# gmlwns2000/sharkshark-4k

Hardware: AMD Instinct MI355X
Metric: upscaled frames/sec at 720p->1440p x2 (whole job) (higher is better)
Workload: dtype f16; 1 GPU; RealESRGAN RRDBNet x2 (23 blocks) 720p->1440p fp16 [BASELINE configs[2]]; io=uint8 NHWC resident in HBM

## Files before the change

### sharkshark-4k_amd/csrc/common.h

```cpp
#pragma once
#include <hip/hip_runtime.h>
#include <hip/hip_fp16.h>
#include <algorithm>
#include <cstdint>
#include <cstdio>
#include <cstdlib>
#include <cstring>
#include <map>
#include <tuple>
#include <set>
#include <string>
#include <vector>
#include <stdexcept>
#include "../../include/ss4k.h"
#ifdef SS4K_DEV
#include "../../include/ss4k_dev.h"
#endif

namespace ss4k {

void set_error(const char* fmt, ...);

struct Error : std::runtime_error {
  int code;
// ... 177 lines not shown

struct ConvArgs {
  const char* in0; size_t in0_plane_bytes; int in0_plane0, nchunks0;
  const char* in1; size_t in1_plane_bytes; int in1_plane0, nchunks1;
  const char* zero_page;
  int N, H, W;
  int n0;
  int job_n;
  float grid_share;
  int mb_override;
  int wide_rl;
  int wide;
  int no_band;
  int ups2;
  int ups_presum;
  const void* wpk;
  const void* w16;
  const float* bias;
  const float* prelu;
  int prelu_le1;
  int act; float slope;
  float alpha, gamma;
  const char* res1; size_t r1_plane_bytes; int r1_plane0;
  const char* res2; size_t r2_plane_bytes; int r2_plane0;
  int bsvd_resid;
  int epi;
  char* out; size_t out_plane_bytes; int out_plane0;
  int cout_real, cout_pad;
  int tiles_x, tiles_y;
  int reverse;
  double flops;
  int dbg;
  unsigned long long* dbg_buf;
};
inline double conv_plane_span_f16(const ConvArgs& a) { return (double)std::max(a.n0 + a.N, a.job_n) * a.H * a.W * 32.0; }
enum { DBG_NO_STORE = 1, DBG_NO_MMA = 2, DBG_NO_TILE_DMA = 4, DBG_NO_W_DMA = 8, DBG_NO_EPILOGUE = 16, DBG_STAMP = 32 };

void launch_conv3x3(ss4k_ctx* ctx, const ConvArgs& a, int dtype, hipStream_t st);
struct PairArgs {
  const char* in; size_t in_plane_bytes; int in_plane0, planes_a;
  const char* wA; const float* biasA;
  const char* wB; const float* biasB;
  const char* res; size_t res_plane_bytes; int res_plane0;
  const char* zero_page;
  unsigned long long* dbg_buf;
  char* out; size_t out_plane_bytes; int out_plane0;
  int epi;
  int cout_real;
  int n0, N, H, W, bands;
  float grid_share;
  double flops;
};
inline bool conv3x3_pair_eligible(int planes_a, int cout_pad_a, int nchunks_b, int cout_pad_b) {
  return (planes_a == 1 || planes_a == 2) && cout_pad_a == 32 && nchunks_b == 2 && cout_pad_b == 32;
}
void launch_conv3x3_pair(ss4k_ctx* ctx, const PairArgs& a, hipStream_t st);

struct DenseArgs {
  const char* in0; size_t in0_plane_bytes; int in0_plane0, nchunks0;
  const char* in1; size_t in1_plane_bytes; int in1_plane0, nchunks1;
  const char* w1; const float* bias1;
  const char* w2; const float* bias2;
  float slope;
  char* out1; size_t out1_plane_bytes; int out1_plane0;
  char* out2; size_t out2_plane_bytes; int out2_plane0;
  const char* zero_page;
// ... 4 lines not shown
  unsigned long long* dbg_buf;
};
inline bool conv3x3_dense2_eligible(int nchunks_a, int cout_pad_a, int nchunks_b, int cout_pad_b) {
  return cout_pad_a == 32 && cout_pad_b == 32 && nchunks_b == nchunks_a + 2 && nchunks_a >= 2 && nchunks_a % 2 == 0;
}
struct ConvArgs;
bool conv3x3_wide_eligible(const ConvArgs& a, int dtype);
void launch_conv3x3_wide(ss4k_ctx* ctx, const ConvArgs& a, hipStream_t st);
void launch_conv3x3_dense2(ss4k_ctx* ctx, const DenseArgs& a, hipStream_t st);
bool conv3x3_w16_eligible(const ConvArgs& a, int dtype);
void launch_conv3x3_w16(ss4k_ctx* ctx, const ConvArgs& a, hipStream_t st);
bool conv3x3_w16n_eligible(const ConvArgs& a, int dtype);
void launch_conv3x3_w16n(ss4k_ctx* ctx, const ConvArgs& a, hipStream_t st);

inline int conv_cw(int) { return 16; }
inline int cout_pad_of(int cout) { return cout <= 32 ? 32 : (cout + 63) / 64 * 64; }
inline int conv_rec_bytes(int dtype) { return dtype == SS4K_F16 ? 32 : 64; }

struct PackSpec {
  int dtype;
  int cout_real, cin_total;
  std::vector<int> cin_map;
  int nchunks0, nchunks1;
  int ps2;
};
struct PackedConv {
  std::vector<uint8_t> w;
  std::vector<float> bias, prelu;
  int cout_pad, nb, groups;
};
PackedConv pack_conv3x3(const PackSpec& s, const float* w_oihw, const float* bias, const float* prelu);
std::vector<uint8_t> pack_conv3x3_w16(const PackSpec& s, const float* w_oihw, int cout_pad);
std::vector<uint8_t> pack_conv3x3_w16n(const PackSpec& s, const float* w_oihw);
int virt_to_real_cout(const PackSpec& s, int v);

}
```

### sharkshark-4k_amd/csrc/conv_dense.hip

```cpp
#include "common.h"
#include <cmath>
#include "conv_tile.h"

namespace ss4k {
namespace dense {

constexpr int NW = 4, MB = 4, TH = NW * MB;
constexpr int XH = TH + 4, XW = TW + 4;
constexpr int REC = 32, SPR = 2;
constexpr int ROWX = XW * REC;
constexpr int XT_SLOTS = XH * XW * SPR;
constexpr int XT_BYTES = XT_SLOTS * 16;
constexpr int XT_DMA = (XT_SLOTS + 63) / 64;
constexpr int DMA_PER_WAVE = (XT_DMA + NW - 1) / NW;
constexpr int WU = 6 * 1024, NSLOT = 5;
constexpr int NDMA = 11;
constexpr int W_OFF = 2 * XT_BYTES, B_OFF = W_OFF + NSLOT * WU, R_OFF = B_OFF + 64 * 4;
constexpr size_t LDS_BYTES = R_OFF + 64 * NW * 4;
static_assert(2 * LDS_BYTES <= 160 * 1024, "two workgroups per CU");
static_assert((TH + 3) * ROWX <= XT_BYTES, "x_k's plane image fits a tile buffer");

__constant__ uint32_t RING_TAB[128] = {
  0x10000, 0x10f00, 0x11000, 0x11500, 0x10300, 0x10400, 0x10600, 0x10a00, 0x11d00, 0x11e00, 0x10005, 0x12106, 0x11600, 0x11900, 0x12100, 0x10003,
  0x12107, 0x1000a, 0x1000c, 0x10511, 0x12108, 0x10009, 0x10111, 0x10611, 0x11311, 0x11611, 0x11d11, 0x00000, 0x10911, 0x10a11, 0x10b11, 0x11111,
// ... 331 lines not shown
      }
    }
    stamp(10);
    if (next_tile < 0) break;
    tile = next_tile; ++kt;
  }
  if constexpr (STAMP) {
    if (lane == 0 && a.dbg_buf && blockIdx.x < 1024) {
      unsigned long long* o = a.dbg_buf + ((size_t)blockIdx.x * 4 + wave) * 16;
      for (int k = 0; k < 11; ++k) o[k] = ph[k];
      o[11] = (unsigned long long)(kt + 1);
      o[12] = ((__builtin_amdgcn_s_memtime() - ct0) << 20) / (__builtin_amdgcn_s_memrealtime() - rt0 + 1);
    }
  }
}

}

namespace wide {

constexpr int NW = 4, MB = 4, TH = NW * MB;
constexpr int XH = TH + 2, XW = TW + 2;
constexpr int REC = 32, SPR = 2;
constexpr int ROWX = XW * REC;
constexpr int XT_SLOTS = XH * XW * SPR;
constexpr int XT_BYTES = XT_SLOTS * 16;
constexpr int XT_DMA = (XT_SLOTS + 63) / 64;
constexpr int DMA_PER_WAVE = (XT_DMA + NW - 1) / NW;
constexpr int WU = 6 * 1024, NSLOT = 6;
constexpr int NDMA = DMA_PER_WAVE + 5;
constexpr int W_OFF = 2 * XT_BYTES, B_OFF = W_OFF + NSLOT * WU;
constexpr size_t LDS_BYTES = B_OFF + 2 * 64 * 4;
static_assert(2 * LDS_BYTES <= 160 * 1024, "two workgroups per CU");

template <bool UPS, bool RL = false>
__global__ __launch_bounds__(64 * NW, 2) void conv3x3_wide_kernel(const ConvArgs a) {
  extern __shared__ __attribute__((aligned(16))) char smem[];
  const uint32_t lds0 = (uint32_t)(size_t)(__attribute__((address_space(3))) char*)smem;
  const int tid = threadIdx.x, lane = tid & 63;
  const int wave = __builtin_amdgcn_readfirstlane(tid >> 6);
  const int lr = lane & 31, lh = lane >> 5;
  const int grp = blockIdx.y;
  const int K = a.nchunks0 + a.nchunks1;
  const int ntiles = a.N * a.tiles_y * a.tiles_x;
  const char* wbase = reinterpret_cast<const char*>(a.wpk) + (size_t)grp * K * (3 * WU);
  const int Hs = a.ups2 ? (a.H >> 1) : a.H, Ws = a.ups2 ? (a.W >> 1) : a.W;

  const bool banded = (gridDim.x % 8 == 0) && ntiles >= (int)gridDim.x && !a.no_band;
  const int tpx = (ntiles + 7) / 8;
  auto tile_of = [&](int k) -> int {
    if (!banded) {
      const int t = blockIdx.x + k * gridDim.x;
      return t < ntiles ? (a.reverse ? ntiles - 1 - t : t) : -1;
    }
    const int base = (blockIdx.x & 7) * tpx, len = min(tpx, ntiles - base);
    const int j = (blockIdx.x >> 3) + k * (gridDim.x >> 3);
    return j < len ? base + (a.reverse ? len - 1 - j : j) : -1;
  };
  auto swz = [](int x) { return (x >> 3) & 1; };
  int rd_base[3];
#pragma unroll
  for (int dx = 0; dx < 3; ++dx) { const int c = lr + dx; rd_base[dx] = (((wave * MB) * XW + c) * SPR + (lh ^ swz(c))) * 16; }

  uint32_t src_off[DMA_PER_WAVE];
  auto setup_tile = [&](int tile, int& n, int& y0, int& x0) {
    const int tx = tile % a.tiles_x, tyn = tile / a.tiles_x;
// ... 229 lines not shown
            }
            __builtin_amdgcn_sched_barrier(0);
            float v[16], r1[16], r2[16];
#pragma unroll
            for (int hq = 0; hq < 2; ++hq) {
              load8<__half>(reinterpret_cast<const char*>(&r1v[hq]), r1 + 8 * hq);
              load8<__half>(reinterpret_cast<const char*>(&r2v[hq]), r2 + 8 * hq);
            }
#pragma unroll
            for (int i = 0; i < 16; ++i) {
              float t = acc[nb][mb][i];
              const float neg = t * slope_v[i];
              t = t >= 0.f ? t : neg;
              if (a.act == ACT_RELU6) t = fminf(t, 6.f);
              t = t * alpha + r1[i];
              v[i] = t * gamma + r2[i];
            }
            if (ok) {
              char* o = outp + rec;
              store8<__half>(o, v);
              store8<__half>(o + a.out_plane_bytes, v + 8);
            }
            __builtin_amdgcn_sched_barrier(0);
          }
        }
        __builtin_amdgcn_sched_barrier(0);
      }
    }
    if (next_tile < 0) break;
    tile = next_tile; ++kt;
  }
}

}

bool conv3x3_wide_eligible(const ConvArgs& a, int dtype) {
  return dtype == SS4K_F16 && a.epi == EPI_NHWC && !a.bsvd_resid && !a.dbg && a.cout_pad >= 64 && a.cout_pad % 64 == 0 &&
         conv_plane_span_f16(a) < 4294967296.0 && (!a.ups2 || (a.H % 2 == 0 && a.W % 2 == 0));
}

void launch_conv3x3_wide(ss4k_ctx* ctx, const ConvArgs& a0, hipStream_t st) {
  using namespace wide;
  ConvArgs a = a0;
  a.tiles_x = (a.W + TW - 1) / TW; a.tiles_y = (a.H + TH - 1) / TH;
  a.zero_page = ctx->zero_page();
  const int groups = a.cout_pad / 64;
  const int ntiles = a.N * a.tiles_y * a.tiles_x;
  const int gx = std::min(ntiles, std::max(1, (int)(ctx->num_cu * 2 / groups * (a.grid_share > 0.f ? a.grid_share : 1.f))));
  auto go = [&](auto kern) {
    const void* fn = reinterpret_cast<const void*>(kern);
    if (ctx->lds_attr_set.insert(fn).second)
      SS4K_HIP(hipFuncSetAttribute(fn, hipFuncAttributeMaxDynamicSharedMemorySize, (int)LDS_BYTES));
    hipLaunchKernelGGL(kern, dim3(gx, groups), dim3(64 * NW), LDS_BYTES, st, a);
  };
  const bool alpha_exact = a.alpha != 0.f && std::fabs(__half2float(__float2half(1.f / a.alpha)) * a.alpha - 1.f) <= 1.2e-7f;
  const bool rl = a.wide_rl && a.res1 && a.act == ACT_NONE && alpha_exact && a.nchunks0 == 4 && a.cout_pad == 64 && !a.ups2 &&
                  a.res1 + (size_t)a.r1_plane0 * a.r1_plane_bytes == a.in0 + (size_t)a.in0_plane0 * a.in0_plane_bytes &&
                  a.r1_plane_bytes == a.in0_plane_bytes;
  ctx->prof_family = rl ? "wide::conv3x3_wide_kernel<RL> (64-cout tile, 32x32x16 MFMA, residual through the matrix core)"
                     : (a.ups2 && a.ups_presum) ? "wide::conv3x3_wide_kernel<UPS> (64-cout tile, 32x32x16 MFMA, nearest-x2 input, pre-summed row taps)"
                                                : "wide::conv3x3_wide_kernel (64-cout tile, 32x32x16 MFMA)";
  if (rl) go(&conv3x3_wide_kernel<false, true>);
  else if (a.ups2 && a.ups_presum) go(&conv3x3_wide_kernel<true>);
  else go(&conv3x3_wide_kernel<false>);
  SS4K_HIP(hipGetLastError());
}

void launch_conv3x3_dense2(ss4k_ctx* ctx, const DenseArgs& a0, hipStream_t st) {
  using namespace dense;
  DenseArgs a = a0;
  SS4K_REQUIRE(a.N > 0 && a.H > 0 && a.W > 0, "dense pair: empty grid");
  SS4K_REQUIRE((a.nchunks0 + a.nchunks1) % 2 == 0 && a.nchunks0 + a.nchunks1 >= 2, "dense pair: conv_k needs an even number of K-chunks");
  SS4K_REQUIRE(a.slope >= 0.f && a.slope <= 1.f, "dense pair: LeakyReLU slope must be in [0,1]");
  SS4K_REQUIRE((double)(a.n0 + a.N) * a.H * a.W * 32.0 < 4294967296.0, "dense pair: a plane holds at most 4 GB");
  a.tiles_x = (a.W + TW - 1) / TW; a.tiles_y = (a.H + TH - 1) / TH;
  a.zero_page = ctx->zero_page();
  const int ntiles = a.N * a.tiles_y * a.tiles_x;
  int gx = std::min(ntiles, std::max(1, (int)(ctx->num_cu * 2 * (a.grid_share > 0.f ? a.grid_share : 1.f))));
#ifdef SS4K_DEV
  if (const char* e = std::getenv("SS4K_DENSE_GRID")) gx = std::min(ntiles, std::max(1, std::atoi(e)));
#endif
  ProfScope prof(ctx, st, PROF_CONV);
  auto go = [&](auto kern) {
    const void* fn = reinterpret_cast<const void*>(kern);
    if (ctx->lds_attr_set.insert(fn).second)
      SS4K_HIP(hipFuncSetAttribute(fn, hipFuncAttributeMaxDynamicSharedMemorySize, (int)LDS_BYTES));
    hipLaunchKernelGGL(kern, dim3(gx), dim3(64 * NW), LDS_BYTES, st, a);
  };
#ifdef SS4K_DEV
  static const bool stamp_mode = std::getenv("SS4K_DENSE_STAMP") && std::getenv("SS4K_DENSE_STAMP")[0] == '1';
  if (stamp_mode) {
    static unsigned long long* dbuf = nullptr;
    if (!dbuf) SS4K_HIP(hipMalloc(reinterpret_cast<void**>(&dbuf), 1024 * 4 * 16 * 8));
    SS4K_HIP(hipMemsetAsync(dbuf, 0, 1024 * 4 * 16 * 8, st));
    a.dbg_buf = dbuf;
    go(&conv3x3_dense2_kernel<0, true>);
// ... 39 lines not shown
```

### sharkshark-4k_amd/csrc/models.cpp

```cpp
#include "models.h"
#include <algorithm>
#include <cmath>
#include <cstdlib>
#include <cstring>

namespace ss4k {

static size_t esz(int dtype) { return dtype == SS4K_F16 ? 2 : 4; }
static int pad16(int c) { return (c + 15) / 16 * 16; }


static std::vector<std::pair<int, int>> bsvd_denblock_shapes(const int* chns, int in_ch, int out_ch, int interm) {
  const int c0 = chns[0], c1 = chns[1], c2 = chns[2];
  return {{interm, in_ch}, {c0, interm}, {c1, c0}, {c1, c1}, {c1, c1}, {c2, c1}, {c2, c2}, {c2, c2},
          {c2, c2}, {c2, c2}, {c1 * 4, c2}, {c1, c1}, {c1, c1}, {c0 * 4, c1}, {c0, c0}, {out_ch, c0}};
}

static void validate_desc(const ss4k_model_desc& d);

size_t model_param_count(const ss4k_model_desc& d) {
  try { validate_desc(d); } catch (const Error&) { return 0; }
  switch (d.kind) {
    case SS4K_FSRCNN:
      return 56 * 25 + 56 + 56 + 12 * 56 + 12 + 12 + 4 * (12 * 12 * 9 + 12 + 12) + 56 * 12 + 56 + 56 + 56 * 81 + 1;
// ... 38 lines not shown
  SS4K_REQUIRE(d.bsvd_stream == 0 || (d.bsvd_stream == 1 && d.kind == SS4K_BSVD), "desc.bsvd_stream is 0 or 1 and only applies to BSVD");
  switch (d.kind) {
    case SS4K_FSRCNN:
      SS4K_REQUIRE(d.scale == 2 || d.scale == 4, "FSRCNN scale must be 2 or 4");
      break;
    case SS4K_RRDBNET:
      SS4K_REQUIRE(d.scale == 1 || d.scale == 2 || d.scale == 4, "RRDBNet scale must be 1, 2 or 4");
      SS4K_REQUIRE(width(d.num_feat, 32), "RRDBNet: num_feat must be a multiple of 32 in 32..512");
      SS4K_REQUIRE(width(d.num_grow_ch, 32), "RRDBNet: num_grow_ch must be a multiple of 32 in 32..512");
      SS4K_REQUIRE(d.num_block > 0 && d.num_block <= MAX_BLOCKS, "RRDBNet: num_block must be in 1..64");
      break;
    case SS4K_SRVGG:
      SS4K_REQUIRE(d.scale == 2 || d.scale == 4, "SRVGG upscale must be 2 or 4 (PixelShuffle tail)");
      SS4K_REQUIRE(width(d.num_feat, 16), "SRVGG: num_feat must be a multiple of 16 in 16..512");
      SS4K_REQUIRE(d.num_block >= 0 && d.num_block <= MAX_BLOCKS, "SRVGG: num_block must be in 0..64");
      break;
    case SS4K_BSVD:
      SS4K_REQUIRE(width(d.bsvd_chns[0], 32), "BSVD: bsvd_chns[0] must be a multiple of 32 in 32..512");
      SS4K_REQUIRE(width(d.bsvd_chns[1], 64), "BSVD: bsvd_chns[1] must be a multiple of 64 in 64..512");
      SS4K_REQUIRE(width(d.bsvd_chns[2], 64), "BSVD: bsvd_chns[2] must be a multiple of 64 in 64..512");
      SS4K_REQUIRE(width(d.bsvd_mid_ch, 32), "BSVD: bsvd_mid_ch must be a multiple of 32 in 32..512");
      SS4K_REQUIRE(d.bsvd_interm_ch > 0 && d.bsvd_interm_ch <= 256, "BSVD: bsvd_interm_ch must be in 1..256");
      break;
    default:
      throw Error(SS4K_EINVAL, "unknown model kind");
  }
}

static void upload(DevBuf& b, const void* src, size_t bytes) {
  b.ensure(std::max<size_t>(bytes, 16));
  SS4K_HIP(hipMemcpy(b.ptr, src, bytes, hipMemcpyHostToDevice));
}

int Model::add_conv(ParamCursor& pc, int cout, int cin_total, PackSpec s, bool has_prelu_after) {
  s.dtype = desc.dtype; s.cout_real = cout; s.cin_total = cin_total;
  const float* w = pc.take((size_t)cout * cin_total * 9);
  const float* b = pc.take(cout);
  const float* a = has_prelu_after ? pc.take(cout) : nullptr;
  PackedConv p = pack_conv3x3(s, w, b, a);
  ConvLayer L;
  upload(L.w, p.w.data(), p.w.size());
  upload(L.bias, p.bias.data(), p.bias.size() * 4);
  if (a) upload(L.prelu, p.prelu.data(), p.prelu.size() * 4);
  if (use_w16 && use_wide && desc.dtype == SS4K_F16 && p.nb == 2 && p.cout_pad % 64 == 0 && (s.nchunks0 + s.nchunks1) % 2 == 0 && !s.ps2) {
    const std::vector<uint8_t> w6 = pack_conv3x3_w16(s, w, p.cout_pad);
    upload(L.w16, w6.data(), w6.size());
    weight_bytes += w6.size();
  }
  if (use_w16 && desc.dtype == SS4K_F16 && cout <= 4 && (s.nchunks0 + s.nchunks1) % 2 == 0 && !s.ps2) {
    const std::vector<uint8_t> w6 = pack_conv3x3_w16n(s, w);
    upload(L.w16, w6.data(), w6.size());
    weight_bytes += w6.size();
  }
  L.has_prelu = a != nullptr;
  if (a) { L.prelu_le1 = true; for (int c = 0; c < cout; ++c) L.prelu_le1 = L.prelu_le1 && a[c] <= 1.f; }
  L.cout_real = cout; L.cout_pad = p.cout_pad; L.nchunks0 = s.nchunks0; L.nchunks1 = s.nchunks1;
  L.cin_real = 0;
  for (int c : s.cin_map) L.cin_real += c >= 0;
  weight_bytes += p.w.size() + p.bias.size() * 4;
  layers.push_back(std::move(L));
  return (int)layers.size() - 1;
}

PackSpec Model::spec_plain(int cin_real, int ps2) const {
  PackSpec s{}; s.ps2 = ps2; s.nchunks0 = planes_for(cin_real); s.nchunks1 = 0;
  s.cin_map.assign((size_t)s.nchunks0 * cw(), -1);
  for (int j = 0; j < cin_real; ++j) s.cin_map[j] = j;
  return s;
}
PackSpec Model::spec_concat(int c0, int c1) const {
  PackSpec s{}; s.nchunks0 = planes_for(c0); s.nchunks1 = planes_for(c1);
  s.cin_map.assign((size_t)(s.nchunks0 + s.nchunks1) * cw(), -1);
  for (int j = 0; j < c0; ++j) s.cin_map[j] = j;
  for (int j = 0; j < c1; ++j) s.cin_map[(size_t)s.nchunks0 * cw() + j] = c0 + j;
  return s;
}
PackSpec Model::spec_masked(int c) const {
  PackSpec s{}; const int first = (c / 4) / cw();
  s.nchunks0 = planes_for(c) - first; s.nchunks1 = 0;
  s.cin_map.assign((size_t)s.nchunks0 * cw(), -1);
  for (int j = 0; j < s.nchunks0 * cw(); ++j) {
    const int ch = first * cw() + j;
    if (ch >= c / 4 && ch < c) s.cin_map[j] = ch;
  }
  return s;
// ... 79 lines not shown
    if (!fs_exact) {
      std::vector<float> scaled = blob;
      float* B = scaled.data();
      for (const Act& A : acts)
        for (int c = 0; c < A.channels; ++c) {
          const float sl = B[off[A.a] + c], sa = 0.5f * (1.f + sl);
          for (int i = 0; i < A.count; ++i) B[off[A.w] + c + (size_t)i * A.stride] *= sa;
          B[off[A.b] + c] *= sa;
          B[off[A.a] + c] = (1.f - sl) / (1.f + sl);
        }
      bool fits = std::fabs(fsw.b_deconv) < 6.0e4f;
      for (float v : scaled) fits = fits && std::fabs(v) < 6.0e4f;
      if (fits) { blob.swap(scaled); fsw.prelu_abs = true; }
      else fs_exact = true;
    }
    upload(fs_blob, blob.data(), blob.size() * 4);
    weight_bytes = blob.size() * 4;
    const float* d = fs_blob.as<float>(); k = 0;
    fsw.w_feat = d + off[k++]; fsw.b_feat = d + off[k++]; fsw.a_feat = d + off[k++];
    fsw.w_shrink = d + off[k++]; fsw.b_shrink = d + off[k++]; fsw.a_shrink = d + off[k++];
    for (int l = 0; l < 4; ++l) { fsw.w_map[l] = d + off[k++]; fsw.b_map[l] = d + off[k++]; fsw.a_map[l] = d + off[k++]; }
    fsw.w_expand = d + off[k++]; fsw.b_expand = d + off[k++]; fsw.a_expand = d + off[k++];
    fsw.w_deconv = d + off[k++];
  } else if (desc.kind == SS4K_RRDBNET) {
    const int nf = desc.num_feat, g = desc.num_grow_ch;
    const int cin0 = 3 * (desc.scale == 2 ? 4 : desc.scale == 1 ? 16 : 1);
    add_conv(pc, nf, cin0, spec_plain(cin0), false);
    for (int b = 0; b < desc.num_block; ++b)
      for (int r = 0; r < 3; ++r)
        for (int c = 0; c < 5; ++c) {
          const int co = c < 4 ? g : nf;
          add_conv(pc, co, nf + c * g, c == 0 ? spec_plain(nf) : spec_concat(nf, c * g), false);
        }
    for (int i = 0; i < 4; ++i) add_conv(pc, nf, nf, spec_plain(nf), false);
    add_conv(pc, 3, nf, spec_plain(nf), false);
  } else if (desc.kind == SS4K_SRVGG) {
    const int nf = desc.num_feat;
    add_conv(pc, nf, 3, spec_plain(3), true);
    for (int i = 0; i < desc.num_block; ++i) add_conv(pc, nf, nf, spec_plain(nf), true);
    add_conv(pc, 3 * desc.scale * desc.scale, nf, spec_plain(nf), false);
  } else {
    for (int blk = 0; blk < 2; ++blk) {
      const int ci = blk == 0 ? 4 : desc.bsvd_mid_ch, co = blk == 0 ? desc.bsvd_mid_ch : 3;
      auto shapes = bsvd_denblock_shapes(desc.bsvd_chns, ci, co, desc.bsvd_interm_ch);
      for (size_t i = 0; i < shapes.size(); ++i) {
        const int cout = shapes[i].first, cin = shapes[i].second;
        const bool masked = (i == 3 || i == 4 || i == 6 || i == 7 || i == 8 || i == 9 || i == 11 || i == 12);
        const bool ps2 = (i == 10 || i == 13);
        add_conv(pc, cout, cin, masked ? (desc.bsvd_stream ? spec_shifted(cin) : spec_masked(cin)) : spec_plain(cin, ps2 ? 1 : 0), false);
      }
    }
  }
  SS4K_REQUIRE(pc.pos == n, "internal: weight cursor did not consume the blob");
}

template <typename Args, typename Launch>
void Model::launch_lanes(Args& a, double flops_per_frame, int N, hipStream_t st, Launch launch) {
  if (ctx->prof && !section_open) {
    section = ctx->prof_get_events();
    SS4K_HIP(hipEventRecord(section.a, st));
    section_open = true;
  }
  if (cur_lanes <= 1 || N != cur_n) {
    a.n0 = 0; a.N = N; a.flops = flops_per_frame * N;
    launch(a, st);
    return;
  }
  if (!forked) {
    SS4K_HIP(hipEventRecord(ctx->lane_fork(), st));
    SS4K_HIP(hipStreamWaitEvent(ctx->lane_stream(), ctx->lane_fork(), 0));
    forked = true;
  }
  for (int l = 0; l < 2; ++l) {
    a.n0 = N * l / 2; a.N = N * (l + 1) / 2 - a.n0;
    a.grid_share = lane_grid_share;
    a.flops = flops_per_frame * a.N;
    launch(a, l == 0 ? st : ctx->lane_stream());
  }
}

void Model::conv(int li,const Tens& in0, const Tens* in1, int N, int H, int W, const ConvOpts& o, hipStream_t st) {
  if (plan_only) return;
#ifdef SS4K_DEV
  if (fail_at_conv > 0 && ++conv_calls == fail_at_conv) throw Error(SS4K_EINVAL, "injected failure (SS4K_FAIL_AT_CONV)");
#endif
  const ConvLayer& L = layers[li];
  ConvArgs a{};
  a.in0 = in0.p; a.in0_plane_bytes = in0.plane_bytes; a.in0_plane0 = in0.plane0; a.nchunks0 = L.nchunks0;
  if (in1) { a.in1 = in1->p; a.in1_plane_bytes = in1->plane_bytes; a.in1_plane0 = in1->plane0; a.nchunks1 = L.nchunks1; }
  SS4K_REQUIRE((in1 != nullptr) == (L.nchunks1 > 0), "internal: conv segment mismatch");
  a.N = N; a.job_n = N; a.H = H; a.W = W; a.ups2 = o.ups2;
  a.wpk = L.w.ptr; a.w16 = L.w16.ptr; a.bias = L.bias.as<float>(); a.prelu = L.has_prelu ? L.prelu.as<float>() : nullptr; a.prelu_le1 = L.prelu_le1 ? 1 : 0;
  a.act = o.act; a.slope = o.slope; a.alpha = o.alpha; a.gamma = o.gamma;
  if (o.res1) { a.res1 = o.res1->p; a.r1_plane_bytes = o.res1->plane_bytes; a.r1_plane0 = o.res1->plane0; }
  if (o.res2) { a.res2 = o.res2->p; a.r2_plane_bytes = o.res2->plane_bytes; a.r2_plane0 = o.res2->plane0; }
  a.bsvd_resid = o.bsvd_resid;
  a.epi = o.epi; a.out = o.out.p; a.out_plane_bytes = o.out.plane_bytes; a.out_plane0 = o.out.plane0;
  a.cout_real = L.cout_real; a.cout_pad = L.cout_pad;
  a.dbg = dbg; a.dbg_buf = dbg_buf; a.mb_override = mb_override; a.wide = use_wide ? 1 : 0; a.ups_presum = ups_presum ? 1 : 0; a.wide_rl = wide_rl ? 1 : 0;
#ifdef SS4K_DEV
  static const bool no_band = std::getenv("SS4K_NO_BAND") && std::getenv("SS4K_NO_BAND")[0] == '1';
  a.no_band = no_band ? 1 : 0;
#endif
  a.reverse = (flip_walk && (launch_parity ^= 1)) ? 1 : 0;
  const double flops = 2.0 * 9.0 * L.cin_real * L.cout_real * (double)H * W * (o.epi == EPI_NHWC_SUB2 ? 0.25 : 1.0);
  if (use_wide && !no_rl && a.res1 && a.act == ACT_NONE && a.nchunks0 == 4 && a.cout_pad == 64 && !a.ups2 &&
      a.res1 + (size_t)a.r1_plane0 * a.r1_plane_bytes == a.in0 + (size_t)a.in0_plane0 * a.in0_plane_bytes) {
    a.wide_rl = 1;
  }
  launch_lanes(a, flops, N, st, [&](const ConvArgs& la, hipStream_t s) { launch_conv3x3(ctx, la, desc.dtype, s); });
}

bool Model::conv_pair(int li, const Tens& in0, int N, int H, int W, const ConvOpts& o, hipStream_t st) {
  const ConvLayer& A = layers[li]; const ConvLayer& B = layers[li + 1];
  const bool plain_b = o.epi == EPI_NHWC && o.act == ACT_RELU6 && !o.res1 && !o.res2 && !o.bsvd_resid;
  const bool resid_b = (o.epi == EPI_NHWC || o.epi == EPI_NCHW_F32) && o.act == ACT_NONE && o.res1 && !o.res2 && o.bsvd_resid && o.alpha == 1.f;
  if (!use_pair || desc.dtype != SS4K_F16 || dbg || o.ups2 || !(plain_b || resid_b) || A.nchunks1 || B.nchunks1 || A.has_prelu || B.has_prelu ||
      !conv3x3_pair_eligible(A.nchunks0, A.cout_pad, B.nchunks0, B.cout_pad) || (o.epi == EPI_NCHW_F32 && B.cout_real > 8))
    return false;
  if (plan_only) return true;
#ifdef SS4K_DEV
  if (fail_at_conv > 0 && ++conv_calls == fail_at_conv) throw Error(SS4K_EINVAL, "injected failure (SS4K_FAIL_AT_CONV)");
#endif
  PairArgs a{};
  a.in = in0.p; a.in_plane_bytes = in0.plane_bytes; a.in_plane0 = in0.plane0; a.planes_a = A.nchunks0;
// ... 472 lines not shown
```

### sharkshark-4k_amd/csrc/models.h

```cpp
#pragma once
#include "common.h"
#include "glue.h"
#include <tuple>

namespace ss4k {

struct Tens { char* p; size_t plane_bytes; int plane0; };

struct ConvLayer {
  DevBuf w, bias, prelu;
  DevBuf w16;
  bool has_prelu = false;
  bool prelu_le1 = false;
  int cout_real = 0, cout_pad = 0, cin_real = 0, nchunks0 = 0, nchunks1 = 0;
};

struct ConvOpts {
  int ups2 = 0;
  int act = ACT_NONE; float slope = 0.f;
  float alpha = 1.f, gamma = 1.f;
  const Tens* res1 = nullptr; const Tens* res2 = nullptr;
  int bsvd_resid = 0;
  int epi = EPI_NHWC;
  Tens out{nullptr, 0, 0};
};

struct ParamCursor {
  const float* base; size_t n, pos = 0;
  const float* take(size_t k) {
    SS4K_REQUIRE(pos + k <= n, "weight blob shorter than the model's state_dict");
    const float* p = base + pos; pos += k; return p;
  }
};
size_t model_param_count(const ss4k_model_desc& d);

struct Model {
  ss4k_ctx* ctx = nullptr;
  ss4k_model_desc desc{};
  std::vector<ConvLayer> layers;
  std::vector<DevBuf> acts;
  DevBuf fs_blob; FsrcnnWeights fsw{};
  size_t weight_bytes = 0;
  bool flip_walk = true;
  int launch_parity = 0;
// ... 17 lines not shown
  int cur_lanes = 1, cur_n = 0;
  bool forked = false;
  struct LaneTune { int calls = 0, decided = 0; hipEvent_t ev[4][2] = {}; float ms[2] = {}; };
  static constexpr size_t LANE_TUNE_MAX = 64;
  std::map<std::tuple<int, int, int>, LaneTune> lane_tune;
  int tune_step(std::map<std::tuple<int, int, int>, LaneTune>& tab, int n, int h, int w, hipStream_t st);

  hipEvent_t tune_timed = nullptr;
  ProfEvent section{}; bool section_open = false;
  void lanes_begin(int n, int h, int w, hipStream_t st);
  void lanes_join(hipStream_t st, bool end_of_forward);
  int dense_mode = 0;
  bool use_wide = true;
  bool use_w16 = true;
  bool wide_rl = false;
  bool ups_presum = true;
  int dense_mask = 3;
  bool use_pair = true;
  int fail_at_conv = 0, conv_calls = 0, forward_calls = 0;
  int dbg = 0;
  unsigned long long* dbg_buf = nullptr;

  void build(const float* w, size_t n);
  void forward(const float* in, float* out, int n, int h, int w, hipStream_t st);
  void forward_impl(const float* in, float* out, int n, int h, int w, hipStream_t st);
  void abort_forward(hipStream_t st) noexcept;
  void out_shape(int n, int h, int w, int* oc, int* oh, int* ow) const;
  int in_channels() const;
  bool no_rl = false;
  ~Model() {
    for (auto* tab : {&lane_tune}) for (auto& t : *tab) for (auto& pr : t.second.ev) for (auto e : pr) if (e) (void)hipEventDestroy(e);
  }

  int add_conv(ParamCursor& pc, int cout, int cin_total, PackSpec spec, bool has_prelu_after);
  PackSpec spec_plain(int cin_real, int ps2 = 0) const;
  PackSpec spec_concat(int c0, int c1) const;
  PackSpec spec_masked(int c) const;
  PackSpec spec_shifted(int c) const;
  int shifted_planes(int c) const { return std::min(planes_for(c), (c / 4 + cw() - 1) / cw()); }
  int cw() const { return conv_cw(desc.dtype); }
  int rec() const { return conv_rec_bytes(desc.dtype); }
  int planes_for(int channels) const { return (channels + cw() - 1) / cw(); }
  void conv(int li, const Tens& in0, const Tens* in1, int N, int H, int W, const ConvOpts& o, hipStream_t st);
  bool conv_pair(int li, const Tens& in0, int N, int H, int W, const ConvOpts& o, hipStream_t st);
  bool conv_dense(int li, const Tens& in0, const Tens* in1, int N, int H, int W, float slope, const Tens& out1, const Tens& out2, hipStream_t st);
  Tens act(int idx, size_t pixels, int channels);
  Tens act_planes(int idx, size_t pixels, int planes);
  void pack_in(const float* in, const Tens& dst, int nplanes, int n, int c, int h, int w, int r, hipStream_t st);

 private:
  template <typename Args, typename Launch> void launch_lanes(Args& a, double flops_per_frame, int N, hipStream_t st, Launch launch);
};

}

namespace ss4k {
double bench_conv_layer(ss4k_ctx* ctx, int dtype, int cin0, int cin1, int cout, int n, int h, int w, int flags,
                        int iters, hipStream_t st);
}
struct ss4k_model { ss4k::Model m; };
```

### sharkshark-4k_amd/csrc/pack.cpp

```cpp
#include "common.h"
#include <cmath>

namespace ss4k {

static inline uint16_t f32_to_f16_bits(float f) {
  uint32_t x; std::memcpy(&x, &f, 4);
  const uint32_t sign = (x >> 16) & 0x8000u;
  int32_t exp = (int32_t)((x >> 23) & 0xff) - 127 + 15;
  uint32_t man = x & 0x7fffffu;
  if (((x >> 23) & 0xff) == 0xff) return (uint16_t)(sign | 0x7c00u | (man ? 0x200u : 0));
  if (exp >= 31) return (uint16_t)(sign | 0x7c00u);
  if (exp <= 0) {
    if (exp < -10) return (uint16_t)sign;
    man |= 0x800000u;
    const int shift = 14 - exp;
    uint32_t h = man >> shift;
    const uint32_t rem = man & ((1u << shift) - 1), half = 1u << (shift - 1);
    if (rem > half || (rem == half && (h & 1))) ++h;
    return (uint16_t)(sign | h);
  }
  uint32_t h = ((uint32_t)exp << 10) | (man >> 13);
  const uint32_t rem = man & 0x1fffu;
  if (rem > 0x1000u || (rem == 0x1000u && (h & 1))) ++h;
  return (uint16_t)(sign | h);
// ... 20 lines not shown
  p.cout_pad = cout_pad_of(s.cout_real);
  p.groups = p.cout_pad / gw;
  const size_t esz = s.dtype == SS4K_F16 ? 2 : 4;
  const size_t nelem = (size_t)p.groups * nchunks * 9 * KS * p.nb * 64 * E;
  p.w.assign(nelem * esz, 0);
  p.bias.assign(p.cout_pad, 0.f);
  p.prelu.assign(p.cout_pad, 0.f);
  for (int v = 0; v < p.cout_pad; ++v) {
    const int co = virt_to_real_cout(s, v);
    if (co >= 0) { p.bias[v] = bias ? bias[co] : 0.f; p.prelu[v] = prelu ? prelu[co] : 0.f; }
  }
  size_t idx = 0;
  for (int g = 0; g < p.groups; ++g)
    for (int c = 0; c < nchunks; ++c)
      for (int dx = 0; dx < 3; ++dx)
        for (int ks = 0; ks < KS; ++ks)
          for (int dy = 0; dy < 3; ++dy)
            for (int nb = 0; nb < p.nb; ++nb)
              for (int lane = 0; lane < 64; ++lane) {
                const int rho = lane & 31, hk = lane >> 5;
                const int v = (g * p.nb + nb) * 32 + 16 * (rho >> 4) + 8 * ((rho >> 2) & 1) + (rho & 3) + 4 * ((rho >> 3) & 1);
                const int co = virt_to_real_cout(s, v);
                for (int e = 0; e < E; ++e, ++idx) {
                  const int ci = s.cin_map[(size_t)c * CW + (2 * ks + hk) * E + e];
                  float val = 0.f;
                  if (ci >= 0 && co >= 0) val = w[((size_t)co * s.cin_total + ci) * 9 + dy * 3 + dx];
                  if (esz == 2) { const uint16_t h = f32_to_f16_bits(val); std::memcpy(&p.w[idx * 2], &h, 2); }
                  else std::memcpy(&p.w[idx * 4], &val, 4);
                }
              }
  return p;
}

std::vector<uint8_t> pack_conv3x3_w16(const PackSpec& s, const float* w, int cout_pad) {
  SS4K_REQUIRE(s.dtype == SS4K_F16, "pack_conv3x3_w16: fp16 only");
  const int nplanes = s.nchunks0 + s.nchunks1;
  SS4K_REQUIRE((int)s.cin_map.size() == nplanes * 16 && nplanes % 2 == 0 && cout_pad % 64 == 0, "pack_conv3x3_w16: shape");
  const int groups = cout_pad / 64, np = nplanes / 2;
  std::vector<uint8_t> out((size_t)groups * np * 3 * 3 * 4 * 64 * 8 * 2, 0);
  size_t idx = 0;
  for (int g = 0; g < groups; ++g)
    for (int q = 0; q < np; ++q)
      for (int ph = 0; ph < 3; ++ph)
        for (int dy = 0; dy < 3; ++dy)
          for (int mbk = 0; mbk < 4; ++mbk)
            for (int lane = 0; lane < 64; ++lane) {
              const int m = lane & 15, kq = lane >> 4, rg = m >> 2, i = m & 3;
              const int co = virt_to_real_cout(s, g * 64 + 32 * (mbk >> 1) + 16 * (rg >> 1) + 8 * (rg & 1) + 4 * (mbk & 1) + i);
              const int plane = ph == 0 ? 2 * q : ph == 1 ? 2 * q + (kq >> 1) : 2 * q + 1;
              const int dx = ph == 1 ? 2 : (kq >> 1);
              for (int e = 0; e < 8; ++e, ++idx) {
                const int ci = s.cin_map[(size_t)plane * 16 + 8 * (kq & 1) + e];
                float val = 0.f;
                if (ci >= 0 && co >= 0) val = w[((size_t)co * s.cin_total + ci) * 9 + dy * 3 + dx];
                const uint16_t h = f32_to_f16_bits(val);
                std::memcpy(&out[idx * 2], &h, 2);
              }
            }
  return out;
}

std::vector<uint8_t> pack_conv3x3_w16n(const PackSpec& s, const float* w) {
  SS4K_REQUIRE(s.dtype == SS4K_F16 && s.cout_real <= 16 && !s.ps2, "pack_conv3x3_w16n: fp16, at most 16 output channels");
  const int nplanes = s.nchunks0 + s.nchunks1;
  SS4K_REQUIRE((int)s.cin_map.size() == nplanes * 16 && nplanes % 2 == 0, "pack_conv3x3_w16n: shape");
  std::vector<uint8_t> out((size_t)(nplanes / 2) * 3 * 3 * 64 * 8 * 2, 0);
// ... 21 lines not shown
```

Before: 120.5 frames/s.

## Add low-resolution LDS tile kernel for nearest-x2 upsample convs with pre-summed row taps

Adds a dedicated kernel for the 3x3 convs that read a nearest-x2 upsampled input. It stages the low-resolution source tile in LDS and uses a host-packed weight blob where adjacent row taps are pre-summed in fp16, so each output row pair needs fewer MFMAs and less tile DMA. The weight blob grows from 6 KB to 8 KB per unit and costs extra device memory. Pre-summing the weights in fp16 can change rounding slightly.

```diff
diff --git a/sharkshark-4k_amd/csrc/common.h b/sharkshark-4k_amd/csrc/common.h
--- a/sharkshark-4k_amd/csrc/common.h
+++ b/sharkshark-4k_amd/csrc/common.h
@@ -233,6 +233,7 @@
   double flops;
   int dbg;
   unsigned long long* dbg_buf;
+  const void* wups;
 };
 inline double conv_plane_span_f16(const ConvArgs& a) { return (double)std::max(a.n0 + a.N, a.job_n) * a.H * a.W * 32.0; }
 enum { DBG_NO_STORE = 1, DBG_NO_MMA = 2, DBG_NO_TILE_DMA = 4, DBG_NO_W_DMA = 8, DBG_NO_EPILOGUE = 16, DBG_STAMP = 32 };
@@ -303,6 +304,8 @@
 PackedConv pack_conv3x3(const PackSpec& s, const float* w_oihw, const float* bias, const float* prelu);
 std::vector<uint8_t> pack_conv3x3_w16(const PackSpec& s, const float* w_oihw, int cout_pad);
 std::vector<uint8_t> pack_conv3x3_w16n(const PackSpec& s, const float* w_oihw);
+std::vector<uint8_t> pack_conv3x3_ups_presum(const PackedConv& p, int nchunks);
+uint16_t f16_add_bits(uint16_t a, uint16_t b);
 int virt_to_real_cout(const PackSpec& s, int v);
 
 }
diff --git a/sharkshark-4k_amd/csrc/conv_dense.hip b/sharkshark-4k_amd/csrc/conv_dense.hip
--- a/sharkshark-4k_amd/csrc/conv_dense.hip
+++ b/sharkshark-4k_amd/csrc/conv_dense.hip
@@ -387,6 +387,97 @@
 constexpr int W_OFF = 2 * XT_BYTES, B_OFF = W_OFF + NSLOT * WU;
 constexpr size_t LDS_BYTES = B_OFF + 2 * 64 * 4;
 static_assert(2 * LDS_BYTES <= 160 * 1024, "two workgroups per CU");
+
+template <bool RL>
+__device__ __forceinline__ void wide_epilogue(const ConvArgs& a, const f32x16 (&acc)[2][MB], const float* epi_lds, int grp, int wave, int lr, int lh,
+                                              int cur_n, int cur_y0, int cur_x0) {
+  const float alpha = a.alpha, gamma = a.gamma;
+  int lhe = lh;
+  asm volatile("" : "+v"(lhe));
+  const int xo = cur_x0 + lr;
+#pragma unroll
+  for (int nb = 0; nb < 2; ++nb) {
+    const int vblock = (grp * 2 + nb) * 32;
+    if (vblock >= a.cout_pad) continue;
+    float slope_v[16];
+#pragma unroll
+    for (int q = 0; q < 4; ++q) {
+      const float4 s4 = *reinterpret_cast<const float4*>(epi_lds + 64 + nb * 32 + 16 * (q >> 1) + 8 * lhe + 4 * (q & 1));
+      slope_v[4 * q] = s4.x; slope_v[4 * q + 1] = s4.y; slope_v[4 * q + 2] = s4.z; slope_v[4 * q + 3] = s4.w;
+    }
+    const int opl = vblock / CW;
+    const size_t sub = (size_t)lhe * 16;
+    const char* r1p = (a.res1 && !RL) ? a.res1 + (size_t)(a.r1_plane0 + opl) * a.r1_plane_bytes + sub : nullptr;
+    const char* r2p = a.res2 ? a.res2 + (size_t)(a.r2_plane0 + opl) * a.r2_plane_bytes + sub : nullptr;
+    char* outp = a.out + (size_t)(a.out_plane0 + opl) * a.out_plane_bytes + sub;
+    const size_t pix0 = ((size_t)cur_n * a.H + cur_y0 + wave * MB) * a.W + xo;
+    if (!r1p && !r2p) {
+      const bool select_form = a.act == ACT_PRELU;
+#pragma unroll
+      for (int mb = 0; mb < MB; ++mb) {
+        const bool ok = (cur_y0 + wave * MB + mb) < a.H && xo < a.W;
+        float v[16];
+        if (a.act == ACT_RELU6) {
+#pragma unroll
+          for (int i = 0; i < 16; ++i) v[i] = fminf(fmaxf(acc[nb][mb][i], 0.f), 6.f) * alpha;
+        } else if (select_form) {
+#pragma unroll
+          for (int i = 0; i < 16; ++i) { const float t = acc[nb][mb][i], neg = t * slope_v[i]; v[i] = (t >= 0.f ? t : neg) * alpha; }
+        } else {
+#pragma unroll
+          for (int i = 0; i < 16; ++i) {
+            const float t = acc[nb][mb][i], st = t * slope_v[i];
+            float mx;
+            asm("v_max_f32 %0, %1, %2" : "=v"(mx) : "v"(t), "v"(st));
+            v[i] = mx * alpha;
+          }
+        }
+        if (ok) {
+          char* o = outp + (pix0 + (size_t)mb * a.W) * REC;
+          store8<__half>(o, v);
+          store8<__half>(o + a.out_plane_bytes, v + 8);
+        }
+      }
+    } else {
+      constexpr int RB = 1;
+#pragma unroll
+      for (int mb0 = 0; mb0 < MB; mb0 += RB) {
+        uint4 r1v[2], r2v[2];
+        const int mb = mb0;
+        const bool ok = (cur_y0 + wave * MB + mb) < a.H && xo < a.W;
+        const size_t rec = (pix0 + (size_t)mb * a.W) * REC;
+#pragma unroll
+        for (int hq = 0; hq < 2; ++hq) {
+          r1v[hq] = (r1p && ok) ? *reinterpret_cast<const uint4*>(r1p + hq * (size_t)a.r1_plane_bytes + rec) : make_uint4(0, 0, 0, 0);
+          r2v[hq] = (r2p && ok) ? *reinterpret_cast<const uint4*>(r2p + hq * (size_t)a.r2_plane_bytes + rec) : make_uint4(0, 0, 0, 0);
+        }
+        __builtin_amdgcn_sched_barrier(0);
+        float v[16], r1[16], r2[16];
+#pragma unroll
+        for (int hq = 0; hq < 2; ++hq) {
+          load8<__half>(reinterpret_cast<const char*>(&r1v[hq]), r1 + 8 * hq);
+          load8<__half>(reinterpret_cast<const char*>(&r2v[hq]), r2 + 8 * hq);
+        }
+#pragma unroll
+        for (int i = 0; i < 16; ++i) {
+          float t = acc[nb][mb][i];
+          const float neg = t * slope_v[i];
+          t = t >= 0.f ? t : neg;
+          if (a.act == ACT_RELU6) t = fminf(t, 6.f);
+          t = t * alpha + r1[i];
+          v[i] = t * gamma + r2[i];
+        }
+        if (ok) {
+          char* o = outp + rec;
+          store8<__half>(o, v);
+          store8<__half>(o + a.out_plane_bytes, v + 8);
+        }
+        __builtin_amdgcn_sched_barrier(0);
+      }
+    }
+    __builtin_amdgcn_sched_barrier(0);
+  }
+}
 
 template <bool UPS, bool RL = false>
 __global__ __launch_bounds__(64 * NW, 2) void conv3x3_wide_kernel(const ConvArgs a) {
@@ -682,6 +773,191 @@
   }
 }
 
+namespace upslr {
+constexpr int LH = TH / 2 + 2, LW = TW / 2 + 2;
+constexpr int ROWX = LW * REC;
+constexpr int XT_SLOTS = LH * LW * SPR;
+constexpr int XT_BYTES = XT_SLOTS * 16;
+constexpr int XT_DMA = (XT_SLOTS + 63) / 64;
+constexpr int DMA_PER_WAVE = (XT_DMA + NW - 1) / NW;
+constexpr int WU = 8 * 1024;
+constexpr int WPIECES = 3 * WU / 1024;
+constexpr int NDMA = DMA_PER_WAVE + WPIECES / NW;
+constexpr int W_OFF = 2 * XT_BYTES, B_OFF = W_OFF + NSLOT * WU;
+constexpr size_t LDS_BYTES = B_OFF + 2 * 64 * 4;
+static_assert(2 * LDS_BYTES <= 160 * 1024, "two workgroups per CU");
+static_assert(TH % 2 == 0 && TW % 2 == 0 && MB == 4, "tile origins and a wave's first row are even; the row table below is for four rows per wave");
+
+__global__ __launch_bounds__(64 * NW, 2) void conv3x3_wide_ups_kernel(const ConvArgs a) {
+  extern __shared__ __attribute__((aligned(16))) char smem[];
+  const uint32_t lds0 = (uint32_t)(size_t)(__attribute__((address_space(3))) char*)smem;
+  const int tid = threadIdx.x, lane = tid & 63;
+  const int wave = __builtin_amdgcn_readfirstlane(tid >> 6);
+  const int lr = lane & 31, lh = lane >> 5;
+  const int grp = blockIdx.y;
+  const int K = a.nchunks0 + a.nchunks1;
+  const int ntiles = a.N * a.tiles_y * a.tiles_x;
+  const char* wbase = reinterpret_cast<const char*>(a.wups) + (size_t)grp * K * (3 * WU);
+  const int Hs = a.H >> 1, Ws = a.W >> 1;
+
+  const bool banded = (gridDim.x % 8 == 0) && ntiles >= (int)gridDim.x && !a.no_band;
+  const int tpx = (ntiles + 7) / 8;
+  auto tile_of = [&](int k) -> int {
+    if (!banded) {
+      const int t = blockIdx.x + k * gridDim.x;
+      return t < ntiles ? (a.reverse ? ntiles - 1 - t : t) : -1;
+    }
+    const int base = (blockIdx.x & 7) * tpx, len = min(tpx, ntiles - base);
+    const int j = (blockIdx.x >> 3) + k * (gridDim.x >> 3);
+    return j < len ? base + (a.reverse ? len - 1 - j : j) : -1;
+  };
+  auto swz = [](int c) { return (c >> 3) & 1; };
+  int rd_base[3];
+#pragma unroll
+  for (int dx = 0; dx < 3; ++dx) { const int c = (lr + dx + 1) >> 1; rd_base[dx] = (((wave * 2) * LW + c) * SPR + (lh ^ swz(c))) * 16; }
+
+  uint32_t src_off[DMA_PER_WAVE];
+  auto setup_tile = [&](int tile, int& n, int& y0, int& x0) {
+    const int tx = tile % a.tiles_x, tyn = tile / a.tiles_x;
+    const int ty = tyn % a.tiles_y;
+    n = a.n0 + tyn / a.tiles_y; y0 = ty * TH; x0 = tx * TW;
+#pragma unroll
+    for (int j = 0; j < DMA_PER_WAVE; ++j) {
+      const int s = (wave + NW * j) * 64 + lane;
+      const int p = s >> 1, gq = s & 1;
+      const int row = p / LW, x = p - row * LW;
+      const int sy = (y0 >> 1) - 1 + row, sx = (x0 >> 1) - 1 + x;
+      const bool ok = s < XT_SLOTS && sy >= 0 && sy < Hs && sx >= 0 && sx < Ws;
+      src_off[j] = ok ? ((uint32_t)(n * Hs + sy) * (uint32_t)Ws + (uint32_t)sx) * REC + (uint32_t)((gq ^ swz(x)) * 16) : OOB;
+    }
+  };
+  auto plane_of = [&](int c) {
+    return (c < a.nchunks0) ? a.in0 + (size_t)(a.in0_plane0 + c) * a.in0_plane_bytes
+                            : a.in1 + (size_t)(a.in1_plane0 + c - a.nchunks0) * a.in1_plane_bytes;
+  };
+  const char* pf_plane = nullptr; const char* pf_w = nullptr; uint32_t pf_tdst = 0; int pf_slot = 0; bool pf_on = false;
+  auto slot_add = [](int s, int k) { const int t = s + k; return t >= NSLOT ? t - NSLOT : t; };
+  auto dma_op = [&](int idx) {
+    if (!pf_on) return;
+    if (idx < DMA_PER_WAVE) {
+      const int k = wave + NW * idx;
+      if (k < XT_DMA) {
+        const char* src = src_off[idx] != OOB ? pf_plane + src_off[idx] : a.zero_page + (lane & 3) * 16;
+        const uint32_t dst = __builtin_amdgcn_readfirstlane(pf_tdst + k * 1024);
+        if (k * 64 + lane < XT_SLOTS) dma16(src, dst);
+      }
+    } else if (idx < NDMA) {
+      const int k = wave + NW * (idx - DMA_PER_WAVE);
+      dma16(pf_w + k * 1024 + lane * 16, __builtin_amdgcn_readfirstlane(lds0 + W_OFF + slot_add(pf_slot, k / 8) * WU + (k % 8) * 1024));
+    }
+  };
+  auto slot_of = [](int g, int m) { return (g < 2 && (m & 1)) ? g * 4 + m / 2 : -1; };
+
+  float* epi_lds = reinterpret_cast<float*>(smem + B_OFF);
+  if (tid < 64) {
+    const int v = grp * 64 + tid;
+    epi_lds[tid] = v < a.cout_pad ? a.bias[v] : 0.f;
+    epi_lds[64 + tid] = a.act == ACT_PRELU ? (v < a.cout_pad ? a.prelu[v] : 1.f) : (a.act == ACT_LRELU ? a.slope : (a.act == ACT_RELU6 ? 0.f : 1.f));
+  }
+
+  int kt = 0;
+  int tile = tile_of(0);
+  if (tile < 0) return;
+  int n, y0, x0;
+  setup_tile(tile, n, y0, x0);
+  int tb = 0, slot = 0;
+  pf_on = true; pf_plane = plane_of(0); pf_tdst = lds0; pf_w = wbase; pf_slot = 0;
+#pragma unroll
+  for (int i = 0; i < NDMA; ++i) dma_op(i);
+  dma_wait();
+  __syncthreads();
+  const int lane16 = lane * 16;
+
+  while (true) {
+    f32x16 acc[2][MB];
+    {
+      typedef float f32x4v __attribute__((ext_vector_type(4)));
+      const uint32_t bl = lds0 + B_OFF + lh * 32;
+#pragma unroll
+      for (int nb = 0; nb < 2; ++nb)
+#pragma unroll
+        for (int mb = 0; mb < MB; ++mb)
+#pragma unroll
+          for (int q = 0; q < 4; ++q) {
+            f32x4v b;
+            asm volatile("ds_read_b128 %0, %1 offset:%2" : "=v"(b) : "v"(bl), "i"(nb * 128 + 64 * (q >> 1) + 16 * (q & 1)));
+            acc[nb][mb][4 * q] = b.x; acc[nb][mb][4 * q + 1] = b.y; acc[nb][mb][4 * q + 2] = b.z; acc[nb][mb][4 * q + 3] = b.w;
+          }
+      asm volatile("s_waitcnt lgkmcnt(0)" ::: "memory");
+    }
+    const int cur_n = n, cur_y0 = y0, cur_x0 = x0;
+    const int next_tile = tile_of(kt + 1);
+
+#pragma unroll 1
+    for (int c = 0; c < K; ++c) {
+      if (c + 1 < K) { pf_on = true; pf_plane = plane_of(c + 1); pf_w = wbase + (size_t)(c + 1) * (3 * WU); }
+      else if (next_tile >= 0) { setup_tile(next_tile, n, y0, x0); pf_on = true; pf_plane = plane_of(0); pf_w = wbase; }
+      else pf_on = false;
+      pf_tdst = lds0 + (tb ^ 1) * XT_BYTES; pf_slot = slot_add(slot, 3);
+      const char* tbp = smem + tb * XT_BYTES;
+      uint4 wf[4][2], af[4];
+      auto af_load = [&](int g, int r) { return *reinterpret_cast<const uint4*>(tbp + rd_base[g] + r * ROWX); };
+      const char* wbp = smem + W_OFF + slot * WU + lane16;
+#pragma unroll
+      for (int f = 0; f < 4; ++f)
+#pragma unroll
+        for (int nb = 0; nb < 2; ++nb) wf[f][nb] = *reinterpret_cast<const uint4*>(wbp + (f * 2 + nb) * 1024);
+#pragma unroll
+      for (int r = 0; r < 4; ++r) af[r] = af_load(0, r);
+#pragma unroll
+      for (int g = 0; g < 3; ++g) {
+        const bool more = g + 1 < 3;
+        const char* wbn = smem + W_OFF + slot_add(slot, g + 1) * WU + lane16;
+        int m = 0;
+        __builtin_amdgcn_sched_barrier(0);
+        __builtin_amdgcn_s_setprio(1);
+#pragma unroll
+        for (int r = 0; r < 4; ++r) {
+          constexpr int NP[4] = {1, 3, 3, 1};
+          constexpr int PMB[4][3] = {{0, 0, 0}, {0, 1, 2}, {1, 2, 3}, {3, 0, 0}};
+          constexpr int PF[4][3] = {{0, 0, 0}, {2, 1, 0}, {3, 2, 1}, {3, 0, 0}};
+#pragma unroll
+          for (int i = 0; i < NP[r]; ++i) {
+            const int mb = PMB[r][i], f = PF[r][i];
+            acc[0][mb] = mma<__half>(wf[f][0], af[r], acc[0][mb]);
+            acc[1][mb] = mma<__half>(wf[f][1], af[r], acc[1][mb]);
+            if (slot_of(g, m) >= 0) {
+              __builtin_amdgcn_sched_barrier(0);
+              dma_op(slot_of(g, m));
+              __builtin_amdgcn_sched_barrier(0);
+            }
+            ++m;
+          }
+          __builtin_amdgcn_sched_barrier(0);
+          if (more) {
+            af[r] = af_load(g + 1, r);
+            if (r == 1) { wf[0][0] = *reinterpret_cast<const uint4*>(wbn); wf[0][1] = *reinterpret_cast<const uint4*>(wbn + 1024); }
+            if (r == 2) {
+              wf[1][0] = *reinterpret_cast<const uint4*>(wbn + 2 * 1024); wf[1][1] = *reinterpret_cast<const uint4*>(wbn + 3 * 1024);
+              wf[2][0] = *reinterpret_cast<const uint4*>(wbn + 4 * 1024); wf[2][1] = *reinterpret_cast<const uint4*>(wbn + 5 * 1024);
+            }
+            if (r == 3) { wf[3][0] = *reinterpret_cast<const uint4*>(wbn + 6 * 1024); wf[3][1] = *reinterpret_cast<const uint4*>(wbn + 7 * 1024); }
+          }
+          __builtin_amdgcn_sched_barrier(0);
+        }
+        __builtin_amdgcn_s_setprio(0);
+      }
+      if (pf_on) { dma_wait(); __syncthreads(); }
+      tb ^= 1; slot = slot_add(slot, 3);
+    }
+
+    wide_epilogue<false>(a, acc, epi_lds, grp, wave, lr, lh, cur_n, cur_y0, cur_x0);
+    if (next_tile < 0) break;
+    tile = next_tile; ++kt;
+  }
+}
+}
+
 }
 
 bool conv3x3_wide_eligible(const ConvArgs& a, int dtype) {
@@ -697,21 +973,32 @@
   const int groups = a.cout_pad / 64;
   const int ntiles = a.N * a.tiles_y * a.tiles_x;
   const int gx = std::min(ntiles, std::max(1, (int)(ctx->num_cu * 2 / groups * (a.grid_share > 0.f ? a.grid_share : 1.f))));
-  auto go = [&](auto kern) {
+  auto go = [&](auto kern, size_t lds = LDS_BYTES) {
     const void* fn = reinterpret_cast<const void*>(kern);
     if (ctx->lds_attr_set.insert(fn).second)
-      SS4K_HIP(hipFuncSetAttribute(fn, hipFuncAttributeMaxDynamicSharedMemorySize, (int)LDS_BYTES));
-    hipLaunchKernelGGL(kern, dim3(gx, groups), dim3(64 * NW), LDS_BYTES, st, a);
+      SS4K_HIP(hipFuncSetAttribute(fn, hipFuncAttributeMaxDynamicSharedMemorySize, (int)lds));
+    hipLaunchKernelGGL(kern, dim3(gx, groups), dim3(64 * NW), lds, st, a);
   };
   const bool alpha_exact = a.alpha != 0.f && std::fabs(__half2float(__float2half(1.f / a.alpha)) * a.alpha - 1.f) <= 1.2e-7f;
   const bool rl = a.wide_rl && a.res1 && a.act == ACT_NONE && alpha_exact && a.nchunks0 == 4 && a.cout_pad == 64 && !a.ups2 &&
                   a.res1 + (size_t)a.r1_plane0 * a.r1_plane_bytes == a.in0 + (size_t)a.in0_plane0 * a.in0_plane_bytes &&
                   a.r1_plane_bytes == a.in0_plane_bytes;
+  const bool ups = a.ups2 && a.ups_presum;
+#ifdef SS4K_DEV
+  static const bool ups_hr_tile = std::getenv("SS4K_UPS_HR_TILE") && std::getenv("SS4K_UPS_HR_TILE")[0] == '1';
+#else
+  constexpr bool ups_hr_tile = false;
+#endif
+  SS4K_REQUIRE(!ups || ups_hr_tile || a.wups, "conv3x3 wide: a pre-summed up-sampling layer needs its blob of weight sums (pack_conv3x3_ups_presum)");
   ctx->prof_family = rl ? "wide::conv3x3_wide_kernel<RL> (64-cout tile, 32x32x16 MFMA, residual through the matrix core)"
-                     : (a.ups2 && a.ups_presum) ? "wide::conv3x3_wide_kernel<UPS> (64-cout tile, 32x32x16 MFMA, nearest-x2 input, pre-summed row taps)"
-                                                : "wide::conv3x3_wide_kernel (64-cout tile, 32x32x16 MFMA)";
+                     : ups ? (ups_hr_tile ? "wide::conv3x3_wide_kernel<UPS> (64-cout tile, 32x32x16 MFMA, nearest-x2 input as an up-sampled LDS tile, row taps summed per tap column)"
+                                          : "wide::conv3x3_wide_kernel<UPS> (64-cout tile, 32x32x16 MFMA, nearest-x2 input as a low-resolution LDS tile, row-tap sums packed)")
+                           : "wide::conv3x3_wide_kernel (64-cout tile, 32x32x16 MFMA)";
   if (rl) go(&conv3x3_wide_kernel<false, true>);
-  else if (a.ups2 && a.ups_presum) go(&conv3x3_wide_kernel<true>);
+#ifdef SS4K_DEV
+  else if (ups && ups_hr_tile) go(&conv3x3_wide_kernel<true>);
+#endif
+  else if (ups) go(&upslr::conv3x3_wide_ups_kernel, upslr::LDS_BYTES);
   else go(&conv3x3_wide_kernel<false>);
   SS4K_HIP(hipGetLastError());
 }
diff --git a/sharkshark-4k_amd/csrc/models.cpp b/sharkshark-4k_amd/csrc/models.cpp
--- a/sharkshark-4k_amd/csrc/models.cpp
+++ b/sharkshark-4k_amd/csrc/models.cpp
@@ -94,7 +94,7 @@
   SS4K_HIP(hipMemcpy(b.ptr, src, bytes, hipMemcpyHostToDevice));
 }
 
-int Model::add_conv(ParamCursor& pc, int cout, int cin_total, PackSpec s, bool has_prelu_after) {
+int Model::add_conv(ParamCursor& pc, int cout, int cin_total, PackSpec s, bool has_prelu_after, bool ups_input) {
   s.dtype = desc.dtype; s.cout_real = cout; s.cin_total = cin_total;
   const float* w = pc.take((size_t)cout * cin_total * 9);
   const float* b = pc.take(cout);
@@ -113,6 +113,11 @@
     const std::vector<uint8_t> w6 = pack_conv3x3_w16n(s, w);
     upload(L.w16, w6.data(), w6.size());
     weight_bytes += w6.size();
+  }
+  if (ups_input && ups_presum && use_wide && desc.dtype == SS4K_F16 && p.nb == 2) {
+    const std::vector<uint8_t> wu = pack_conv3x3_ups_presum(p, s.nchunks0 + s.nchunks1);
+    upload(L.wups, wu.data(), wu.size());
+    weight_bytes += wu.size();
   }
   L.has_prelu = a != nullptr;
   if (a) { L.prelu_le1 = true; for (int c = 0; c < cout; ++c) L.prelu_le1 = L.prelu_le1 && a[c] <= 1.f; }
@@ -258,7 +263,7 @@
           const int co = c < 4 ? g : nf;
           add_conv(pc, co, nf + c * g, c == 0 ? spec_plain(nf) : spec_concat(nf, c * g), false);
         }
-    for (int i = 0; i < 4; ++i) add_conv(pc, nf, nf, spec_plain(nf), false);
+    for (int i = 0; i < 4; ++i) add_conv(pc, nf, nf, spec_plain(nf), false, i == 1 || i == 2);
     add_conv(pc, 3, nf, spec_plain(nf), false);
   } else if (desc.kind == SS4K_SRVGG) {
     const int nf = desc.num_feat;
@@ -316,7 +321,7 @@
   if (in1) { a.in1 = in1->p; a.in1_plane_bytes = in1->plane_bytes; a.in1_plane0 = in1->plane0; a.nchunks1 = L.nchunks1; }
   SS4K_REQUIRE((in1 != nullptr) == (L.nchunks1 > 0), "internal: conv segment mismatch");
   a.N = N; a.job_n = N; a.H = H; a.W = W; a.ups2 = o.ups2;
-  a.wpk = L.w.ptr; a.w16 = L.w16.ptr; a.bias = L.bias.as<float>(); a.prelu = L.has_prelu ? L.prelu.as<float>() : nullptr; a.prelu_le1 = L.prelu_le1 ? 1 : 0;
+  a.wpk = L.w.ptr; a.w16 = L.w16.ptr; a.wups = L.wups.ptr; a.bias = L.bias.as<float>(); a.prelu = L.has_prelu ? L.prelu.as<float>() : nullptr; a.prelu_le1 = L.prelu_le1 ? 1 : 0;
   a.act = o.act; a.slope = o.slope; a.alpha = o.alpha; a.gamma = o.gamma;
   if (o.res1) { a.res1 = o.res1->p; a.r1_plane_bytes = o.res1->plane_bytes; a.r1_plane0 = o.res1->plane0; }
   if (o.res2) { a.res2 = o.res2->p; a.r2_plane_bytes = o.res2->plane_bytes; a.r2_plane0 = o.res2->plane0; }
diff --git a/sharkshark-4k_amd/csrc/models.h b/sharkshark-4k_amd/csrc/models.h
--- a/sharkshark-4k_amd/csrc/models.h
+++ b/sharkshark-4k_amd/csrc/models.h
@@ -10,6 +10,7 @@
 struct ConvLayer {
   DevBuf w, bias, prelu;
   DevBuf w16;
+  DevBuf wups;
   bool has_prelu = false;
   bool prelu_le1 = false;
   int cout_real = 0, cout_pad = 0, cin_real = 0, nchunks0 = 0, nchunks1 = 0;
@@ -93,7 +94,7 @@
     for (auto* tab : {&lane_tune}) for (auto& t : *tab) for (auto& pr : t.second.ev) for (auto e : pr) if (e) (void)hipEventDestroy(e);
   }
 
-  int add_conv(ParamCursor& pc, int cout, int cin_total, PackSpec spec, bool has_prelu_after);
+  int add_conv(ParamCursor& pc, int cout, int cin_total, PackSpec spec, bool has_prelu_after, bool ups_input = false);
   PackSpec spec_plain(int cin_real, int ps2 = 0) const;
   PackSpec spec_concat(int c0, int c1) const;
   PackSpec spec_masked(int c) const;
diff --git a/sharkshark-4k_amd/csrc/pack.cpp b/sharkshark-4k_amd/csrc/pack.cpp
--- a/sharkshark-4k_amd/csrc/pack.cpp
+++ b/sharkshark-4k_amd/csrc/pack.cpp
@@ -76,6 +76,50 @@
   return p;
 }
 
+uint16_t f16_add_bits(uint16_t a, uint16_t b) {
+  const auto special = [](uint16_t h) { return (h & 0x7c00u) == 0x7c00u; };
+  if (special(a) || special(b)) {
+    const bool nan = (special(a) && (a & 0x3ffu)) || (special(b) && (b & 0x3ffu)) || (special(a) && special(b) && ((a ^ b) & 0x8000u));
+    if (nan) return 0x7e00u;
+    return special(a) ? a : b;
+  }
+  const auto fixed = [](uint16_t h) -> int64_t {
+    const int e = (h >> 10) & 0x1f, m = h & 0x3ff;
+    const int64_t v = e ? (int64_t)(1024 + m) << (e - 1) : (int64_t)m;
+    return (h & 0x8000u) ? -v : v;
+  };
+  const int64_t n = fixed(a) + fixed(b);
+  if (n == 0) return (uint16_t)(a & b & 0x8000u);
+  const uint16_t sign = n < 0 ? 0x8000u : 0;
+  const uint64_t mag = (uint64_t)(n < 0 ? -n : n);
+  if (mag < 2048) return (uint16_t)(sign | mag);
+  int p = 63;
+  while (!((mag >> p) & 1)) --p;
+  const int shift = p - 10;
+  uint32_t h = (uint32_t)((p - 9) << 10) + (uint32_t)((mag >> shift) - 1024);
+  const uint64_t rem = mag & ((1ull << shift) - 1), half = 1ull << (shift - 1);
+  if (rem > half || (rem == half && (h & 1))) ++h;
+  return (uint16_t)(sign | (h >= 0x7c00u ? 0x7c00u : h));
+}
+
+std::vector<uint8_t> pack_conv3x3_ups_presum(const PackedConv& p, int nchunks) {
+  SS4K_REQUIRE(p.nb == 2 && p.w.size() == (size_t)p.groups * nchunks * 3 * 6144, "pack_conv3x3_ups_presum: an fp16 blob of 64-cout groups");
+  std::vector<uint8_t> out((size_t)p.groups * nchunks * 3 * 8192);
+  const size_t FR = 2 * 64 * 8;
+  std::vector<uint16_t> w(3 * FR), o(4 * FR);
+  for (size_t u = 0; u < (size_t)p.groups * nchunks * 3; ++u) {
+    std::memcpy(w.data(), &p.w[u * 6144], 6144);
+    for (size_t i = 0; i < FR; ++i) {
+      o[i] = w[i];
+      o[FR + i] = f16_add_bits(w[i], w[FR + i]);
+      o[2 * FR + i] = f16_add_bits(w[FR + i], w[2 * FR + i]);
+      o[3 * FR + i] = w[2 * FR + i];
+    }
+    std::memcpy(&out[u * 8192], o.data(), 8192);
+  }
+  return out;
+}
+
 std::vector<uint8_t> pack_conv3x3_w16(const PackSpec& s, const float* w, int cout_pad) {
   SS4K_REQUIRE(s.dtype == SS4K_F16, "pack_conv3x3_w16: fp16 only");
   const int nplanes = s.nchunks0 + s.nchunks1;
```

After: 120.7 frames/s (median of 2 runs). About the same (+0.2%).
